# ScissorJack-ever/AlayaLite

Hardware: AMD Instinct MI355X
Metric: QPS @ recall@10>=0.95, GIST-960 L2, 1M base / 1k queries (higher is better)
Workload: dtype f32

## Files before the change

### alayalite_amd/csrc/capi.cpp

```cpp
#include "../../include/alaya_hip.h"

#include <hip/hip_runtime_api.h>

#include <algorithm>
#include <cfloat>
#include <cmath>
#include <cstring>
#include <memory>
#include <mutex>
#include <stdexcept>
#include <limits>
#include <string>
#include <thread>
#include <vector>

#include "build_kernels.h"
#include "extend_kernels.h"
#include "graph_update.h"
#include "hnsw_build.h"
#include "flat_bound.h"
#include "flat_filtered_kernels.h"
#include "flat_kernels.h"
#include <cstdlib>
#include "screen_bound.h"
// ... 73 lines not shown
  int device = 0;
  std::mutex mu;
  uint64_t n = 0;
  uint32_t dim = 0, stride = 0;
  int metric = ALAYA_METRIC_L2;
  bool generic = false;
  DevBuf base, valid;
  bool has_valid = false;
  bool has_graph = false;
  uint32_t R = 0, upper_R = 0, ep = 0, n_eps = 0;
  bool has_overlay = false, dedup = false;
  DevBuf l0, levels, upper_off, upper_edges, eps;
  uint64_t graph_n = 0;
  bool has_sq8 = false;
  int sq8_order = 2;
  uint32_t code_stride = 0;
  DevBuf codes, sq_min, sq_max, rr_q_buf, sq_ids, sq_d;
  DevBuf norms, cand_d, cand_i, flat_tau, flag_buf, iota, flat_q;
  DevBuf flat_bias;
  int flat_contraction = -1;
  bool norms_ready = false;
  DevBuf flat_tiles, tiles_cand, tiles_qexp;
  bool tiles_ready = false;
  int tiles_exp = 0;
  int tiles_metric = -1;
  float max_norm = 0.f;
  DevBuf work, overflow, dirty, stab, q_buf, id_buf, dist_buf, cnt_buf, dlist_buf, dout_buf;
  DevBuf allow_buf, group_buf;
  DevBuf through_buf;
  DevBuf ff_ids, ff_sums, ff_count, ff_part_d, ff_part_i, ff_qlist;
  uint64_t ff_last[4] = {0, 0, 0, 0};
  size_t overflow_clean = 0;
  size_t stab_clean = 0;
  uint32_t hash_log2_override = 0;
  int helpers_mode = -1;
  DevBuf help_stats;
  uint64_t help_stats_slots = 0;
  struct ScreenCopy {
    DevBuf rows, err;
    uint64_t cap = 0;
    bool ready = false;
    bool failed = false;
  };
  ScreenCopy screen_copy[2];
  uint32_t screen_format = 0;
  DevBuf screen_stats;
  uint64_t screen_stats_slots = 0;
  uint32_t last_grid = 0, last_waves = 0;
  uint32_t last_lds = 0, last_hash_log2 = 0, last_compact = 0, last_per_cu = 0, last_scout = 0;
  DevBuf scout_stats;
  uint64_t scout_stats_slots = 0;
  DevBuf scout_policy_stats;
  uint32_t last_scout_policy = 0;
  int visited_mode_override = 0;
  int num_cus = 0;
  uint64_t capacity = 0;
  std::unique_ptr<alaya_amd::HostGraph> upd_graph;
  std::unique_ptr<alaya_amd::RowMirror> upd_rows;
  std::unique_ptr<alaya_amd::UpdateContext> upd_ctx;
  hipStream_t stream = nullptr;
  hipEvent_t scratch_ev = nullptr;
  hipStream_t scratch_stream = nullptr;
  bool scratch_used = false;
  uint64_t device_bytes() const {
    return base.bytes + valid.bytes + l0.bytes + levels.bytes + upper_off.bytes +
           upper_edges.bytes + eps.bytes + overflow.bytes + dirty.bytes + stab.bytes + codes.bytes + sq_min.bytes +
           sq_max.bytes;
  }
};

namespace {

void set_device(const alaya_index *ix) { hip_check(hipSetDevice(ix->device), "hipSetDevice"); }

void scratch_acquire(alaya_index *ix, hipStream_t s) {
  if (ix->scratch_used && ix->scratch_stream != s)
    hip_check(hipStreamWaitEvent(s, ix->scratch_ev, 0), "hipStreamWaitEvent");
}
void scratch_release(alaya_index *ix, hipStream_t s) {
  hip_check(hipEventRecord(ix->scratch_ev, s), "hipEventRecord");
  ix->scratch_stream = s;
  ix->scratch_used = true;
}
void scratch_suspect(alaya_index *ix) {
  ix->overflow_clean = 0;
  ix->stab_clean = 0;
}
void scratch_drain(alaya_index *ix) {
  if (!ix->scratch_used) return;
  const hipError_t e = hipEventSynchronize(ix->scratch_ev);
  if (e != hipSuccess) scratch_suspect(ix);
  hip_check(e, "hipEventSynchronize");
}
template <typename F>
int guarded_scratch(alaya_index *ix, F &&f) {
  return guarded([&] {
    try {
      f();
    } catch (const DeviceError &) {
      if (ix) scratch_suspect(ix);
      throw;
    }
  });
}

SearchParams base_params(alaya_index *ix) {
// ... 185 lines not shown
  if (helpers_requested(ix, p, nq, static_cast<uint64_t>(stream_cus(ix, stream))) && ix->R <= 64 &&
      search_has_helpers(ix->dim, p.sq8_order, ix->generic))
    r.want |= kModeHelp;
  const bool plain = (r.want & (kModeHelp | kModeStamp)) == 0;
  if (plain && search_has_two_waves(ix->dim, p.sq8_order, ix->generic)) {
    const char *e = std::getenv("ALAYA_TWO_WAVES");
    const int force = e ? std::atoi(e) : -1;
    if (force == 1) {
      r.want |= kModeTwoWaves;
    } else if (force != 0) {
      int b1 = 0;
      const size_t probe = search_wave_lds_bytes(ix->stride, ef, 12, true);
      hip_check(search_occupancy(resolve_search_variant(r), p.ip, 1, probe, &b1), "occupancy");
      const uint64_t resident1 = static_cast<uint64_t>(std::max(1, b1)) * static_cast<uint64_t>(stream_cus(ix, stream));
      if (nq > resident1 && 2 * nq <= 3 * resident1) r.want |= kModeTwoWaves;
    }
  }
  if (ensure_screen(ix, p, p.sq8_order == 0 && plain, stream)) r.want |= kModeScreen;
  return r;
}

struct SearchPlan {
  const alaya_amd::SearchVariant *variant;
  int W;
  size_t lds;
  int grid;
  int per_cu;
};

uint32_t scout_default(uint32_t dim) { return (dim == 768 || dim == 960) ? alaya_amd::kScoutOn : 0u; }

uint32_t scout_requested(uint32_t dim) {
  const char *e = std::getenv("ALAYA_SEARCH_SCOUT");
  const int asked = e && e[0] ? std::atoi(e) : -1;
  uint32_t f = asked < 0 ? scout_default(dim) : (asked == 1 ? alaya_amd::kScoutOn : (asked == 2 ? alaya_amd::kScoutOn | alaya_amd::kScoutVerify : 0u));
  if (f != 0u) {
    const char *m = std::getenv("ALAYA_SEARCH_SCOUT_MISS");
    if (m && std::atoi(m) != 0) f |= alaya_amd::kScoutMiss;
  }
  return f;
}

uint32_t scout_policy_default(uint32_t dim) {
  return (dim == 768 || dim == 960) ? (alaya_amd::kScoutEarly | alaya_amd::kScoutRecheck) : 0u;
}

uint32_t scout_policy_requested(uint32_t dim) {
  const char *e = std::getenv("ALAYA_SEARCH_SCOUT_POLICY");
  if (!(e && e[0])) return scout_policy_default(dim);
  return static_cast<uint32_t>(std::strtoul(e, nullptr, 0)) &
         (alaya_amd::kScoutEarly | alaya_amd::kScoutRecheck);
}

SearchPlan plan_search(alaya_index *ix, SearchParams &p, alaya_amd::SearchRequest r, uint64_t nq, uint32_t ef,
                       hipStream_t stream) {
  using namespace alaya_amd;
  SearchPlan plan{};
  for (;;) {
    plan.variant = &resolve_search_variant(r);
    const int mode = plan.variant->mode;
    if ((r.want & kModeStamp) != 0 && (mode & kModeStamp) == 0)
      throw ArgError("no stamped search kernel for dim " + std::to_string(ix->dim) +
                     (p.sq8_order ? " SQ8 (order " + std::to_string(p.sq8_order) + ")" : std::string(" f32")) +
                     ": see the variant list in search_variants.h");
    p.help = (mode & kModeHelp) != 0;
    p.two_waves = (mode & kModeTwoWaves) != 0;
    p.screen = (mode & kModeScreen) != 0 ? ix->screen_format : 0u;
    plan.W = p.help ? 4 : search_waves(p);
    while (!p.help && plan.W > 1 && static_cast<uint64_t>(plan.W) > nq) plan.W /= 2;
    p.hash_log2 = size_visited(ix, p, *plan.variant, nq, ef, plan.W);
    const bool compact = p.vis_rbits != kVisWide;
    p.wave_lds = static_cast<uint32_t>(search_wave_lds_bytes(ix->stride, ef, p.hash_log2, compact, p.sq8_order));
    bool fits = true;
    if (p.help) {
      const size_t need = static_cast<size_t>(plan.W) * kHelpMemoSlots * ix->R * 8;
      const size_t q_bytes = search_query_lds_bytes(ix->stride, p.sq8_order);
      if (q_bytes >= need) {
        p.memo_off = 0;
      } else if (p.wave_lds >= q_bytes + 3 * 64 * 4 + need) {
        p.memo_off = static_cast<uint32_t>(q_bytes + 3 * 64 * 4);
      } else {
        fits = false;
      }
    }
    plan.lds = search_shared_lds_bytes(ix->stride, p.sq8_order != 0) + static_cast<size_t>(plan.W) * p.wave_lds +
               (p.help ? kHelpBoardBytes : 0);
    if (!p.help || (fits && plan.lds <= kLdsPerCu)) break;
    r.want &= ~kModeHelp;
  }
  if (plan.lds > kLdsPerCu) throw ArgError("ef / dim too large for the LDS budget");
  int per_cu = 0;
  hip_check(search_occupancy(*plan.variant, p.ip, plan.W, plan.lds, &per_cu), "occupancy");
  per_cu = static_cast<int>(std::max<uint64_t>(1, std::min<uint64_t>(per_cu, max_search_waves_per_cu() / plan.W)));
  const uint64_t cus = static_cast<uint64_t>(stream_cus(ix, stream));
  const uint64_t blocks_needed = p.help ? static_cast<uint64_t>(per_cu) * cus : (nq + plan.W - 1) / plan.W;
  plan.grid = static_cast<int>(std::max<uint64_t>(1, std::min<uint64_t>(blocks_needed, static_cast<uint64_t>(per_cu) * cus)));
  plan.per_cu = per_cu;
  p.scout = 0u;
  p.scout_policy = 0u;
  const uint32_t scout = scout_requested(ix->dim);
  if (scout != 0u && p.screen == 3u && !p.ip && !p.two_waves && !p.help && plan.W == 1 && ix->R <= kScoutR &&
      (plan.variant->mode & ~kModeScreen) == 0 && search_has_two_waves(ix->dim, p.sq8_order, ix->generic) &&
      !helpers_requested(ix, p, nq, cus)) {
    SearchRequest r2 = r;
    r2.want |= kModeTwoWaves;
    const SearchVariant &v2 = resolve_search_variant(r2);
    const size_t lds2 = plan.lds + kScoutBoardBytes;
    int per_cu2 = 0;
    if (v2.mode == (kModeScreen | kModeTwoWaves) && lds2 <= kLdsPerCu)
      hip_check(search_occupancy(v2, false, 2, lds2, &per_cu2), "occupancy");
    if (per_cu2 >= per_cu && nq <= static_cast<uint64_t>(per_cu) * cus) {
      plan.variant = &v2;
      plan.lds = lds2;
      p.scout = scout;
      p.scout_policy = scout_policy_requested(ix->dim);
      if (const char *e = std::getenv("ALAYA_SEARCH_SCOUT_GRID"))
        plan.grid = std::max(1, std::min(plan.grid, std::atoi(e)));
    }
  }
  return plan;
}

SearchParams graph_search_params(alaya_index *ix, const float *d_q, uint64_t nq, uint32_t k, uint32_t ef, uint32_t *d_ids,
                                 float *d_dists, uint32_t *d_cnt) {
  SearchParams p = base_params(ix);
  p.l0 = ix->l0.as<uint32_t>();
  p.R = ix->R;
  p.dedup_edges = ix->dedup;
  p.levels = ix->has_overlay ? ix->levels.as<uint32_t>() : nullptr;
  p.upper_off = ix->upper_off.as<uint64_t>();
  p.upper_edges = ix->upper_edges.as<uint32_t>();
  p.upper_R = ix->upper_R;
  p.ep = ix->ep;
  p.eps = ix->eps.as<uint32_t>();
  p.n_eps = ix->n_eps;
  p.queries = d_q;
  p.nq = nq;
  p.q_stride = ix->dim;
  p.k = k;
  p.ef = ef;
  p.out_ids = d_ids;
  p.out_dists = d_dists;
  p.out_counters = d_cnt;
  return p;
}

void set_search_space(alaya_index *ix, SearchParams &p, bool sq8, uint32_t ef) {
  if (sq8) {
    p.sq8_order = ix->sq8_order;
    p.codes = ix->codes.as<uint8_t>();
    p.code_stride = ix->code_stride;
    p.sq_min = ix->sq_min.as<float>();
    p.sq_max = ix->sq_max.as<float>();
  }
  p.stab_log2 = spill_table_log2(p.sq8_order, std::max<uint32_t>(1, ceil_log2(std::max<uint64_t>(ix->n, 2))), ef);
}

void record_launch(alaya_index *ix, SearchParams &p, int grid, int wg_waves, size_t lds, int per_cu, uint64_t searchers,
                   hipStream_t stream) {
  ix->last_grid = static_cast<uint32_t>(grid);
  ix->last_waves = static_cast<uint32_t>(wg_waves);
  ix->last_lds = static_cast<uint32_t>(lds);
  ix->last_hash_log2 = p.hash_log2;
  ix->last_compact = p.vis_rbits != alaya_amd::kVisWide ? 1u : 0u;
  ix->last_per_cu = static_cast<uint32_t>(per_cu);
  ix->last_scout = p.scout;
  ix->last_scout_policy = p.scout_policy;
  ix->scout_stats_slots = p.scout ? searchers : 0;
  ix->help_stats_slots = p.help ? searchers : 0;
  ix->screen_stats_slots = p.screen ? searchers : 0;
  ix->work.reserve(4);
  p.work_counter = ix->work.as<uint32_t>();
  hip_check(hipMemsetAsync(p.work_counter, 0, 4, stream), "hipMemsetAsync");
}

void do_search(alaya_index *ix, const float *d_q, uint64_t nq, uint32_t k, uint32_t ef,
               uint32_t *d_ids, float *d_dists, uint32_t *d_cnt, hipStream_t stream,
               uint64_t *d_stamps = nullptr, bool sq8 = false, uint32_t fill_id = 0) {
  if (!ix->base.ptr) throw ArgError("index has no base vectors");
  if (!ix->has_graph) throw ArgError("index has no graph");
  if (ef == 0) throw ArgError("ef must be >= 1");
  if (k == 0 || nq == 0) return;
  if (ix->graph_n > ix->n) throw ArgError("graph has more nodes than base vectors");
  SearchParams p = graph_search_params(ix, d_q, nq, k, ef, d_ids, d_dists, d_cnt);
  p.stamps = d_stamps;
  p.fill_id = fill_id;
  if (sq8 && !ix->has_sq8) throw ArgError("index has no SQ8 codes");
  set_search_space(ix, p, sq8, ef);
  if (const char *e = std::getenv("ALAYA_HELP_FLAGS")) p.help_flags = static_cast<uint32_t>(std::strtoul(e, nullptr, 10));
  const SearchPlan plan = plan_search(ix, p, search_request(ix, p, nq, ef, stream), nq, ef, stream);
  if (p.screen >= 2) {
    p.screen_u8 = ix->screen_copy[1].rows.as<uint8_t>();
  } else if (p.screen) {
    p.screen_rows = ix->screen_copy[0].rows.as<uint16_t>();
    p.screen_err = ix->screen_copy[0].err.as<float>();
  }
  scratch_acquire(ix, stream);
  const uint64_t searchers = static_cast<uint64_t>(plan.grid) * plan.W;
  prepare_spill(ix, p, searchers, stream);
  const int wg_waves = p.scout ? 2 * plan.W : plan.W;
  if (p.scout) {
    ix->scout_stats.reserve(searchers * 16);
    p.scout_stats = ix->scout_stats.as<uint32_t>();
    ix->scout_policy_stats.reserve(searchers * 12);
    p.scout_policy_stats = ix->scout_policy_stats.as<uint32_t>();
  }
  if (p.help) {
    ix->help_stats.reserve(searchers * 12);
    p.help_stats = ix->help_stats.as<uint32_t>();
  }
  if (p.screen) {
    ix->screen_stats.reserve(searchers * 8);
    p.screen_stats = ix->screen_stats.as<uint32_t>();
  }
  record_launch(ix, p, plan.grid, wg_waves, plan.lds, plan.per_cu, searchers, stream);
  hip_check(alaya_amd::launch_search(*plan.variant, p, plan.grid, wg_waves, plan.lds, stream), "search launch");
  scratch_release(ix, stream);
}

void do_filtered_search(alaya_index *ix, const float *d_q, uint64_t nq, uint32_t k, uint32_t ef, const uint32_t *d_allow,
// ... 1985 lines not shown
    if (waves_per_group) *waves_per_group = ix->last_waves;
  });
}

int alaya_index_last_plan(const alaya_index *ix, uint32_t *lds_bytes, uint32_t *hash_log2, uint32_t *compact,
                          uint32_t *groups_per_cu, uint32_t *scout) {
  return guarded([&] {
    if (!ix) throw ArgError("null index");
    if (lds_bytes) *lds_bytes = ix->last_lds;
    if (hash_log2) *hash_log2 = ix->last_hash_log2;
    if (compact) *compact = ix->last_compact;
    if (groups_per_cu) *groups_per_cu = ix->last_per_cu;
    if (scout) *scout = ix->last_scout;
  });
}

static std::vector<uint64_t> searcher_stats(alaya_index *ix, const DevBuf &buf, uint64_t searchers, uint32_t words) {
  std::vector<uint64_t> t(words, 0);
  if (searchers) {
    set_device(ix);
    scratch_drain(ix);
    std::vector<uint32_t> h(words * searchers);
    hip_check(hipMemcpy(h.data(), buf.ptr, h.size() * 4, hipMemcpyDeviceToHost), "D2H");
    for (uint64_t i = 0; i < h.size(); ++i) t[i % words] += h[i];
  }
  return t;
}

int alaya_index_scout_stats(alaya_index *ix, uint64_t *expansions, uint64_t *hits, uint64_t *records,
                            uint64_t *mismatches) {
  return guarded_scratch(ix, [&] {
    if (!ix) throw ArgError("null index");
    const std::vector<uint64_t> t = searcher_stats(ix, ix->scout_stats, ix->scout_stats_slots, 4);
    if (expansions) *expansions = t[0];
    if (hits) *hits = t[1];
    if (records) *records = t[2];
    if (mismatches) *mismatches = t[3];
  });
}

int alaya_index_scout_policy_stats(alaya_index *ix, uint32_t *policy, uint64_t *early_posts, uint64_t *confirmed,
                                   uint64_t *abandoned) {
  return guarded_scratch(ix, [&] {
    if (!ix) throw ArgError("null index");
    const bool sums = early_posts || confirmed || abandoned;
    const std::vector<uint64_t> t = searcher_stats(ix, ix->scout_policy_stats, sums ? ix->scout_stats_slots : 0, 3);
    if (policy) *policy = ix->last_scout_policy;
    if (early_posts) *early_posts = t[0];
    if (confirmed) *confirmed = t[1];
    if (abandoned) *abandoned = t[2];
  });
}

int alaya_index_set_helpers(alaya_index *ix, int mode) {
  return guarded([&] {
    if (!ix) throw ArgError("null index");
    if (mode < -1 || mode > 1) throw ArgError("helpers mode must be -1 (automatic), 0 (off) or 1 (on)");
    ix->helpers_mode = mode;
  });
}

int alaya_index_help_stats(alaya_index *ix, uint64_t *memo_dists, uint64_t *memo_expansions, uint64_t *helper_rows) {
  return guarded_scratch(ix, [&] {
    if (!ix) throw ArgError("null index");
    const std::vector<uint64_t> t = searcher_stats(ix, ix->help_stats, ix->help_stats_slots, 3);
    if (memo_dists) *memo_dists = t[0];
    if (memo_expansions) *memo_expansions = t[1];
    if (helper_rows) *helper_rows = t[2];
  });
}

int alaya_screen_lower_bound(const float *d_tilde, const float *e_row, uint64_t n, uint32_t dim, float *out) {
  return guarded([&] {
    if (n && (!d_tilde || !e_row || !out)) throw ArgError("invalid arguments");
    for (uint64_t i = 0; i < n; ++i) out[i] = alaya_amd::screen_lower_bound(d_tilde[i], e_row[i], dim);
  });
}

namespace {
void screen_u8_quantize_one(const float *x, uint32_t dim, uint8_t *codes, float *header, float *values) {
  using namespace alaya_amd;
  float lo = FLT_MAX, hi = -FLT_MAX;
  bool bad = false;
  for (uint32_t j = 0; j < dim; ++j) {
    bad = bad || !screen_finite(x[j]);
    lo = fminf(lo, x[j]);
    hi = fmaxf(hi, x[j]);
  }
  float scale = screen_u8_scale(lo, hi);
  if (bad || !screen_finite(scale)) {
    bad = true;
    lo = scale = 0.f;
  }
  float sum = 0.f;
  for (uint32_t j = 0; j < dim; ++j) {
    const uint32_t c = screen_u8_code(x[j], lo, scale);
    const float y = screen_u8_value(c, lo, scale);
    const float d = x[j] - y;
    if (!bad) sum = fmaf(d, d, sum);
    codes[j] = static_cast<uint8_t>(c);
    if (values) values[j] = y;
  }
  header[0] = screen_u8_err(sum, dim, bad);
  header[1] = lo;
  header[2] = scale;
  header[3] = 0.f;
// ... 115 lines not shown
```

### alayalite_amd/csrc/pybind_module.cpp

```cpp
#include <pybind11/numpy.h>
#include <pybind11/pybind11.h>
#include <pybind11/stl.h>

#include <algorithm>
#include <cmath>
#include <cstring>
#include <fstream>
#include <memory>
#include <queue>
#include <stdexcept>
#include <string>
#include <vector>

#include "../../include/alaya_hip.h"

extern "C" int alaya_index_flat_diag(alaya_index *, const float *, uint64_t, uint32_t, int, uint32_t *, float *,
                                     uint32_t *, uint32_t *, void *);
#include "host_distance.h"

namespace py = pybind11;

namespace alaya_py {

enum class IndexType { FLAT = 0, HNSW = 1, NSG = 2, FUSION = 3, QG = 4 };
// ... 105 lines not shown
                           eps.mutable_data()));
  return py::make_tuple(l0, has_overlay ? py::object(levels) : py::none(), has_overlay ? py::object(off) : py::none(), ue,
                        ep, upper_R, eps);
}

class LaunchControls {
 public:
  void set_hash_log2(uint32_t v) { check(alaya_index_set_hash_log2(ix_, v)); }
  void set_visited_mode(int m) { check(alaya_index_set_visited_mode(ix_, m)); }
  void set_helpers(int m) { check(alaya_index_set_helpers(ix_, m)); }
  py::tuple last_launch() {
    uint32_t g = 0, w = 0;
    check(alaya_index_last_launch(ix_, &g, &w));
    return py::make_tuple(g, w);
  }
  py::tuple help_stats() {
    uint64_t m = 0, x = 0, r = 0;
    check(alaya_index_help_stats(ix_, &m, &x, &r));
    return py::make_tuple(m, x, r);
  }
  py::tuple screen_stats() {
    uint64_t a = 0, b = 0;
    check(alaya_index_screen_stats(ix_, &a, &b));
    return py::make_tuple(a, b);
  }
  py::tuple scout_stats() {
    uint64_t e = 0, h = 0, r = 0, m = 0;
    check(alaya_index_scout_stats(ix_, &e, &h, &r, &m));
    return py::make_tuple(e, h, r, m);
  }
  py::tuple scout_policy_stats() {
    uint64_t a = 0, c = 0, d = 0;
    check(alaya_index_scout_policy_stats(ix_, nullptr, &a, &c, &d));
    return py::make_tuple(a, c, d);
  }
  uint32_t scout_policy() {
    uint32_t pol = 0;
    check(alaya_index_scout_policy_stats(ix_, &pol, nullptr, nullptr, nullptr));
    return pol;
  }
  py::dict last_plan() {
    uint32_t g = 0, w = 0, lds = 0, hl = 0, c = 0, pc = 0, sc = 0;
    check(alaya_index_last_launch(ix_, &g, &w));
    check(alaya_index_last_plan(ix_, &lds, &hl, &c, &pc, &sc));
    py::dict d;
    d["workgroups"] = g;
    d["waves_per_group"] = w;
    d["lds_bytes"] = lds;
    d["hash_log2"] = hl;
    d["compact"] = c != 0;
    d["groups_per_cu"] = pc;
    d["scout"] = sc;
    d["scout_policy"] = scout_policy();
    return d;
  }

 protected:
  alaya_index *ix_ = nullptr;
};

class PyIndexInterface : public LaunchControls {
 public:
  explicit PyIndexInterface(const IndexParams &params) : params_(params) {
    dtype_ = dtype_code(params_.data_type_);
    if (params_.id_type_.is(py::dtype::of<uint32_t>())) {
      id_bytes_ = 4;
    } else if (params_.id_type_.is(py::dtype::of<uint64_t>())) {
      id_bytes_ = 8;
    } else {
      throw std::runtime_error("Unsupported id type");
    }
    if (params_.quantization_type_ == QuantizationType::SQ4 ||
        params_.quantization_type_ == QuantizationType::RABITQ)
      throw std::runtime_error("quantization type not supported by the MI355X engine (SQ4/RaBitQ are out of scope)");
    if (params_.metric_ == MetricType::COS && dtype_ != kF32 && dtype_ != kF64) {
      throw std::runtime_error("COS metric only support float or double");
    }
    if (params_.quantization_type_ == QuantizationType::SQ8 && dtype_ != kF32)
      throw std::runtime_error("SQ8 quantization of non-float32 data is not supported by the MI355X engine");
    check(alaya_index_create(0, &ix_));
  }
  ~PyIndexInterface() {
    if (graph_) alaya_graph_free(graph_);
    if (ix_) alaya_index_destroy(ix_);
  }
  PyIndexInterface(const PyIndexInterface &) = delete;
  PyIndexInterface &operator=(const PyIndexInterface &) = delete;

  std::string to_string() const { return "PyIndexInterface"; }

  void fit(py::array vectors, uint32_t ef_construction, uint32_t num_threads, const std::string &builder) {
    if (builder != "host" && builder != "gpu") throw py::value_error("builder must be 'host' or 'gpu'");
    if (vectors.ndim() != 2) throw std::runtime_error("Array must be 2D");
    check_dtype(vectors);
    py::array arr = py::array::ensure(vectors, py::array::c_style);
    const uint64_t n = arr.shape(0);
    dim_ = static_cast<uint32_t>(arr.shape(1));
    if (n > params_.capacity_) throw std::runtime_error("number of vectors exceeds the index capacity");
    if (params_.metric_ == MetricType::COS) normalize_in_place(arr, n);
    raw_.assign(static_cast<const char *>(arr.data()),
                static_cast<const char *>(arr.data()) + n * dim_ * dtype_size(dtype_));
    n_ = n;
    delete_cnt_ = 0;
    valid_.clear();
    rows_f32_.resize(n * dim_);
    to_float(raw_.data(), dtype_, n * dim_, rows_f32_.data());
// ... 1147 lines not shown
```

### alayalite_amd/csrc/search_device.h

```cpp
#pragma once
#include <hip/hip_runtime.h>

#include <cfloat>
#include <cstdint>

#include "screen_bound.h"
#include "search_kernels.h"

namespace alaya_amd {
namespace {

constexpr uint32_t kEmpty = 0xffffffffu;
constexpr uint32_t kChecked = 0x80000000u;
constexpr uint32_t kIdMask = 0x7fffffffu;

__device__ __forceinline__ int lane_id() { return __lane_id(); }

__device__ __forceinline__ void wave_sync() {
  __builtin_amdgcn_fence(__ATOMIC_SEQ_CST, "wavefront");
  __builtin_amdgcn_wave_barrier();
}

__device__ __forceinline__ uint64_t ballot(bool p) { return __ballot(p); }

// ... 1160 lines not shown
  if (lane_in_row && row_v != kEmpty)
    lo = __hip_atomic_load(&vs.bits[row_v >> 5], __ATOMIC_RELAXED, __HIP_MEMORY_SCOPE_AGENT);
}

__device__ __forceinline__ void visit_end(Visited &vs) {
  if (!vs.spilled) return;
  const int lane = lane_id();
  __threadfence_block();
  if (vs.stab != nullptr) {
    uint64_t *t = reinterpret_cast<uint64_t *>(vs.stab);
    const uint32_t n8 = 2u * (vs.stab_bmask + 1u);
    for (uint32_t i = lane; i < n8; i += 64) __hip_atomic_store(t + i, 0ull, __ATOMIC_RELAXED, ALAYA_STAB_SCOPE);
  }
  if (vs.ndirty <= vs.dirty_cap) {
    for (uint32_t i = lane; i < vs.ndirty; i += 64)
      __hip_atomic_store(&vs.bits[vs.dirty[i]], 0u, __ATOMIC_RELAXED, __HIP_MEMORY_SCOPE_AGENT);
  } else {
    for (uint64_t w = lane; w < vs.n_words; w += 64)
      __hip_atomic_store(&vs.bits[w], 0u, __ATOMIC_RELAXED, __HIP_MEMORY_SCOPE_AGENT);
  }
  stab_order();
  vs.spilled = false;
}

struct PoolState {
  uint32_t size;
  uint32_t cur;
  uint32_t ef;
};

__device__ __forceinline__ uint32_t pool_upper_bound(const float *pd, uint32_t size, float d) {
  uint32_t lo = 0, hi = size;
  while (lo < hi) {
    const uint32_t mid = (lo + hi) >> 1;
    if (pd[mid] > d) hi = mid; else lo = mid + 1;
  }
  return lo;
}

__device__ __forceinline__ uint32_t batch_lower_bound(const float *sd, uint32_t n, float d) {
  uint32_t lo = 0, hi = n;
  while (lo < hi) {
    const uint32_t mid = (lo + hi) >> 1;
    if (sd[mid] < d) lo = mid + 1; else hi = mid;
  }
  return lo;
}

struct NoNext {
  __device__ void operator()(uint32_t) const {}
};

struct NoMark {
  __device__ void operator()() const {}
};

template <bool kRegMerge = false, typename OnNext = NoNext, typename Mark = NoMark>
__device__ void pool_merge(PoolState &ps, const Lds &L, bool has, uint32_t id, float d,
                           OnNext on_next = OnNext(), Mark mark = Mark()) {
  const int lane = lane_id();
  const bool full = ps.size == ps.ef;
  const float last = full ? L.pd[ps.size - 1] : 0.f;
  const bool acc = has && !(full && d >= last);
  const uint64_t amask = ballot(acc);
  const uint32_t n_acc = __popcll(amask);
  if (n_acc == 0) return;
  if (kRegMerge && ps.ef <= 128) {
    const uint32_t size = ps.size;
    const bool v0 = static_cast<uint32_t>(lane) < size;
    const bool v1 = static_cast<uint32_t>(lane) + 64 < size;
    const float p0 = v0 ? L.pd[lane] : 0.f;
    const float p1 = v1 ? L.pd[lane + 64] : 0.f;
    const uint32_t i0 = v0 ? L.pi[lane] : 0u;
    const uint32_t i1 = v1 ? L.pi[lane + 64] : 0u;
    if (!ballot((acc && d != d) || (v0 && p0 != p0) || (v1 && p1 != p1))) {
      uint32_t rank = 0, pos = 0, s0 = 0, s1 = 0;
      uint64_t rest = amask;
      while (rest) {
        const int j = __ffsll(static_cast<unsigned long long>(rest)) - 1;
        rest &= rest - 1;
        const float dj = read_lane(d, j);
        rank += (dj < d || (dj == d && j < lane)) ? 1u : 0u;
        const uint32_t ub = __popcll(ballot(v0 && p0 <= dj)) + __popcll(ballot(v1 && p1 <= dj));
        if (lane == j) pos = ub;
        s0 += dj < p0 ? 1u : 0u;
        s1 += dj < p1 ? 1u : 0u;
      }
      pos += rank;
      const int lane0 = __ffsll(static_cast<unsigned long long>(ballot(acc && rank == 0))) - 1;
      const uint32_t first_pos = read_lane(pos, lane0);
      if (first_pos <= ps.cur) on_next(read_lane(id, lane0));
      mark();
      wave_sync();
      if (v0 && s0 != 0 && lane + s0 < ps.ef) {
        L.pd[lane + s0] = p0;
        L.pi[lane + s0] = i0;
      }
      if (v1 && s1 != 0 && lane + 64 + s1 < ps.ef) {
        L.pd[lane + 64 + s1] = p1;
        L.pi[lane + 64 + s1] = i1;
      }
      if (acc && pos < ps.ef) {
        L.pd[pos] = d;
        L.pi[pos] = id;
      }
      wave_sync();
      ps.size = min(size + n_acc, ps.ef);
      if (first_pos < ps.cur) ps.cur = first_pos;
      return;
    }
  }
  uint32_t rank = 0;
  uint64_t rest = amask;
#if ALAYA_PAIR_LOOPS
  while (rest) {
    const int j = __ffsll(static_cast<unsigned long long>(rest)) - 1;
    rest &= rest - 1;
    const bool t2 = rest != 0ull;
    const int j2 = t2 ? __ffsll(static_cast<unsigned long long>(rest)) - 1 : j;
    rest &= t2 ? rest - 1 : rest;
    const float dj = read_lane(d, j);
    const float dj2 = read_lane(d, j2);
    rank += (dj < d || (dj == d && j < lane)) ? 1u : 0u;
    rank += (t2 && (dj2 < d || (dj2 == d && j2 < lane))) ? 1u : 0u;
  }
#else
  while (rest) {
    const int j = __ffsll(static_cast<unsigned long long>(rest)) - 1;
    rest &= rest - 1;
    const float dj = read_lane(d, j);
    rank += (dj < d || (dj == d && j < lane)) ? 1u : 0u;
  }
#endif
  if (acc) L.sd[rank] = d;
  uint32_t pos = 0;
  if (acc) pos = pool_upper_bound(L.pd, ps.size, d) + rank;
  const int lane0 = __ffsll(static_cast<unsigned long long>(ballot(acc && rank == 0))) - 1;
  const uint32_t first_pos = read_lane(pos, lane0);
  if (first_pos <= ps.cur) on_next(read_lane(id, lane0));
  mark();
  wave_sync();
  for (int hi = static_cast<int>(ps.size); hi > static_cast<int>(first_pos); hi -= 64) {
    const int j = hi - 64 + lane;
    const bool mv = j >= static_cast<int>(first_pos);
    float pdj = 0.f;
    uint32_t pij = 0;
    uint32_t dest = 0;
    if (mv) {
      pdj = L.pd[j];
      pij = L.pi[j];
      dest = static_cast<uint32_t>(j) + batch_lower_bound(L.sd, n_acc, pdj);
    }
    wave_sync();
    if (mv && dest < ps.ef) {
      L.pd[dest] = pdj;
      L.pi[dest] = pij;
    }
    wave_sync();
  }
  if (acc && pos < ps.ef) {
    L.pd[pos] = d;
    L.pi[pos] = id;
  }
  wave_sync();
  ps.size = min(ps.size + n_acc, ps.ef);
  if (first_pos < ps.cur) ps.cur = first_pos;
}

template <bool kNext = false>
__device__ __forceinline__ uint32_t pool_pop(PoolState &ps, const Lds &L, uint32_t *c1 = nullptr,
                                             uint32_t *c2 = nullptr) {
  const int lane = lane_id();
  const uint32_t raw = L.pi[ps.cur];
  wave_sync();
  if (lane == 0) L.pi[ps.cur] = raw | kChecked;
  uint32_t next = ps.size;
  if constexpr (kNext) *c1 = *c2 = kEmpty;
  for (uint32_t b = ps.cur + 1; b < ps.size; b += 64) {
    const uint32_t j = b + lane;
    const uint32_t pij = j < ps.size ? L.pi[j] : kChecked;
    const bool un = !(pij & kChecked);
    const uint64_t mk = ballot(un);
    if (mk) {
      const int f = __ffsll(static_cast<unsigned long long>(mk)) - 1;
      next = b + f;
      if constexpr (kNext) {
        *c1 = read_lane(pij & kIdMask, f);
        const uint64_t mk2 = mk & (mk - 1ull);
        if (mk2) *c2 = read_lane(pij & kIdMask, __ffsll(static_cast<unsigned long long>(mk2)) - 1);
      }
      break;
    }
  }
  wave_sync();
  ps.cur = next;
  return raw & kIdMask;
}

}
}
```

### alayalite_amd/csrc/search_kernels.h

```cpp
#pragma once
#include <hip/hip_runtime_api.h>

#include <cstddef>
#include <cstdint>

#include "search_variants.h"

namespace alaya_amd {

struct SearchParams {
  const float *base;
  uint64_t n;
  uint32_t dim;
  uint32_t stride;
  const uint32_t *valid;
  bool ip;
  bool generic;
  const uint32_t *l0;
  uint32_t R;
  bool dedup_edges;
  const uint32_t *levels;
  const uint64_t *upper_off;
  const uint32_t *upper_edges;
  uint32_t upper_R;
  uint32_t ep;
  const uint32_t *eps;
  uint32_t n_eps;
  const float *queries;
  uint64_t nq;
  uint32_t q_stride;
  uint32_t k;
  uint32_t ef;
  uint32_t *out_ids;
  float *out_dists;
  uint32_t *out_counters;
  uint32_t fill_id;
  uint32_t *work_counter;
  uint32_t *overflow_bits;
  uint32_t *dirty_words;
  uint32_t dirty_cap;
  uint32_t wave_lds;
  uint32_t hash_log2;
  uint32_t vis_rbits;
  uint32_t vis_lbits;
  uint32_t vis_max_disp;
  uint32_t vis_limit;
  uint16_t *spill_table;
  uint32_t stab_log2;
  uint32_t stab_rbits;
  uint32_t spill_flags;
  uint64_t *stamps;
  int sq8_order;
  const uint8_t *codes;
  uint32_t code_stride;
  const float *sq_min;
  const float *sq_max;
  uint32_t help;
  uint32_t help_flags;
  uint32_t memo_off;
  uint32_t two_waves;
  uint32_t *help_stats;
  uint32_t screen;
  const uint16_t *screen_rows;
  const float *screen_err;
  const uint8_t *screen_u8;
  uint32_t *screen_stats;
  uint32_t scout;
  uint32_t *scout_stats;
  uint32_t scout_policy;
  uint32_t *scout_policy_stats;
};
constexpr uint32_t kScoutOn = 1, kScoutVerify = 2, kScoutMiss = 4;
constexpr uint32_t kScoutEarly = 1, kScoutRecheck = 2;
constexpr uint32_t kScoutSlots = 3;
constexpr uint32_t kScoutR = 32;
constexpr size_t kScoutBoardBytes = kScoutSlots * (kScoutR * 4 + 8 + 4) + 20;

struct FilterParams {
  const uint32_t *allow;
  const uint32_t *mask_of_query;
  uint32_t mask_words;
  uint32_t k;
  uint32_t result_off;
};

struct HopParams {
  uint32_t *n_through;
};

struct RerankParams {
  const uint32_t *search_ids;
  uint32_t k;
  uint32_t n_src;
  uint32_t n_take;
  uint32_t zeros;
  uint32_t fill_id;
  uint32_t *out_ids;
  float *out_dists;
};

constexpr uint32_t kVisWide = 0xffffffffu;
constexpr size_t kHelpBoardBytes = 256;
#ifndef ALAYA_HELP_DEPTH
#define ALAYA_HELP_DEPTH 1
#endif
constexpr size_t kHelpMemoSlots = ALAYA_HELP_DEPTH + 1;
constexpr uint32_t kStabBucket = 8;
inline size_t visited_table_bytes(uint32_t hash_log2, bool compact) {
  return (static_cast<size_t>(compact ? 2 : 4)) << hash_log2;
}
size_t search_wave_lds_bytes(uint32_t stride, uint32_t ef, uint32_t hash_log2, bool compact = false,
                             int sq8_order = 0);
size_t search_query_lds_bytes(uint32_t stride, int sq8_order);
__host__ __device__ inline size_t search_shared_lds_bytes(uint32_t stride, bool sq8) {
  return sq8 ? 2 * static_cast<size_t>(stride) * 4 : 0;
}
hipError_t launch_rerank(const SearchParams &p, const RerankParams &r, hipStream_t stream);
hipError_t search_occupancy(const SearchVariant &v, bool ip, int waves, size_t lds, int *blocks_per_cu);
hipError_t launch_screen_rows(const float *base, uint64_t first, uint64_t count, uint32_t stride,
                              uint16_t *out_rows, float *out_err, hipStream_t stream);
hipError_t launch_screen_rows_u8(const float *base, uint64_t first, uint64_t count, uint32_t stride,
                                 uint8_t *out_recs, hipStream_t stream);
hipError_t launch_search(const SearchVariant &v, const SearchParams &p, int grid, int waves, size_t lds,
                         hipStream_t stream);
size_t filter_result_lds_bytes(uint32_t k);
hipError_t filtered_search_occupancy(uint32_t dim, bool generic, bool ip, int waves, size_t lds, int *blocks_per_cu);
// ... 17 lines not shown
```

### alayalite_amd/csrc/search_kernels.hip

```cpp
#include <hip/hip_runtime.h>

#include <cfloat>
#include <cstdint>

#include "screen_bound.h"
#include "search_kernels.h"
#include "search_device.h"

#ifndef ALAYA_MIN_WAVES_SQ8
#define ALAYA_MIN_WAVES_SQ8 -1
#endif
#ifndef ALAYA_MIN_WAVES_NARROW
#define ALAYA_MIN_WAVES_NARROW 0
#endif
#ifndef ALAYA_MIN_WAVES_WIDE
#define ALAYA_MIN_WAVES_WIDE 0
#endif
template <int kSpace>
constexpr bool space_sq8() { return kSpace == 1 || kSpace == 2; }
template <int kSpace>
constexpr bool space_tab() { return kSpace == 2; }

template <int kChunks, int kSpace, int kMode = 0>
constexpr int search_min_waves() {
// ... 920 lines not shown
            const float4 head = *reinterpret_cast<const float4 *>(rp);
            const uint2 sums = *reinterpret_cast<const uint2 *>(rp + screen_u8_sums_offset(p.stride));
            screen_dots_int<kChunks>(p, sq.codes, L.cid, nf, reinterpret_cast<uint32_t *>(L.cd), second_level_prefetch);
            lb3 = screen_int_bound(p.stride, sq.err, sq.lo, sq.scale, sq.a1, sq.a2, head.x, head.y, head.z, sums.x, sums.y,
                                   __float_as_uint(L.cd[lane]));
          } else if (p.screen == 2) {
            if (in) e_row = *reinterpret_cast<const float *>(p.screen_u8 + static_cast<uint64_t>(c) * screen_u8_record_bytes(p.stride));
            screen_distances_u8<kChunks, kScreenRowsU8>(p, L.q, L.cid, nf, L.cd, second_level_prefetch);
          } else {
            if (in) e_row = p.screen_err[c];
            screen_distances<kChunks, kScreenRows>(p, L.q, L.cid, nf, L.cd, second_level_prefetch);
          }
          bool keep = false;
          if (in) {
            const float lb = p.screen == 3 ? lb3 : screen_lower_bound(L.cd[lane], e_row, p.dim);
            keep = !(lb > 0.f && lb >= tau);
          }
          const uint64_t km = ballot(keep);
          nd = __popcll(km);
          n_screened += static_cast<uint32_t>(nf);
          n_screened_out += static_cast<uint32_t>(nf - nd);
          if constexpr (kScout) {
            if (early && nd > 0 && ps.cur < ps.size) scout_early_request(sboard, L, ps, keep, lb3, c, pred);
          }
          if (keep) L.cid[__popcll(km & ((1ull << lane) - 1ull))] = c;
          wave_sync();
          if (nd == 0) {
            stamp(3);
            n_dist += nf;
            continue;
          }
        }
      }
      if constexpr (kScreen) {
        constexpr int kFull = RowPass<kChunks, kRows>::kR;
        if (nd <= 8) {
          space_distances<kIP, kChunks, kSpace, false, 1>(p, L, L.cid, nd, L.cd);
        } else if (kFull > 2 && nd <= 16) {
          space_distances<kIP, kChunks, kSpace, false, 2>(p, L, L.cid, nd, L.cd);
        } else {
          space_distances<kIP, kChunks, kSpace, false, kRows>(p, L, L.cid, nd, L.cd);
        }
      } else if (!kHelp || compute) {
        space_distances<kIP, kChunks, kSpace, kHelp, kRows>(p, L, dist_ids, nf, L.cd, second_level_prefetch);
      } else {
        second_level_prefetch();
      }
      stamp(3);
      n_dist += nf;
      const bool has = lane < nd;
      const uint32_t cid = has ? L.cid[lane] : 0u;
      const float cd = has ? L.cd[lane] : 0.f;
      wave_sync();
      pool_merge<kRegMerge>(ps, L, has, cid, cd, [&](uint32_t nx) {
        if (nx != pred) {
          const uint32_t old_pred = pred;
          (void)old_pred;
          pred = nx;
          if (lane < static_cast<int>(p.R)) pred_v = p.l0[static_cast<uint64_t>(nx) * p.R + lane];
          if constexpr (kHelp) {
            if (mine.memo_wave >= 0) mine_request(board, wave, mine, kEmpty, nx, old_pred);
          }
          if constexpr (kScout) {
            if (scouting && ps.size == ps.ef) scout_retarget(sboard, early, nx, old_pred);
          }
        }
      }
#ifdef ALAYA_FINE_STAMPS
      , [&]() { stamp(7); }
#endif
      );
      stamp(4);
    }

    query_end(p, L, ps, qi, n_dist, n_expand, n_dist_up, n_hops_up);
    visit_end(vs);
    if constexpr (kStamp) {
      st[6] = __builtin_readcyclecounter() - t_begin;
      if (lane < 8) p.stamps[static_cast<uint64_t>(qi) * 8 + lane] = st[lane & 7];
    }
    wave_sync();
  }
  if constexpr (kHelp) {
    help_siblings<kIP, kChunks, kSpace>(p, smem, L, board, wave, W);
    help_stats_out(p, board, wave, slot, lane);
  }
  if constexpr (kScout) {
    if (scouting) scout_leave(p, sboard, slot);
  }
  if constexpr (kScreen) screen_stats_out(p, slot, n_screened, n_screened_out, lane);
}

__global__ void __launch_bounds__(256) screen_rows_kernel(const float *base, uint64_t first, uint64_t count,
                                                          uint32_t stride, uint16_t *out_rows, float *out_err) {
  const int lane = lane_id();
  const uint64_t waves = static_cast<uint64_t>(gridDim.x) * (blockDim.x >> 6);
  for (uint64_t r = static_cast<uint64_t>(blockIdx.x) * (blockDim.x >> 6) + (threadIdx.x >> 6); r < count; r += waves) {
    const float *row = base + (first + r) * stride;
    uint16_t *dst = out_rows + (first + r) * stride;
    float sum = 0.f;
    bool bad = false;
    for (uint32_t e = 2 * lane; e < stride; e += 128) {
      const float2 x = *reinterpret_cast<const float2 *>(row + e);
      const _Float16 h0 = static_cast<_Float16>(x.x), h1 = static_cast<_Float16>(x.y);
      const float y0 = static_cast<float>(h0), y1 = static_cast<float>(h1);
      bad = bad || !(fabsf(y0) <= 65504.f) || !(fabsf(y1) <= 65504.f) || !(fabsf(x.x) <= FLT_MAX) ||
            !(fabsf(x.y) <= FLT_MAX);
      const float d0 = x.x - y0, d1 = x.y - y1;
      sum = fmaf(d0, d0, sum);
      sum = fmaf(d1, d1, sum);
      const half2_t h = {h0, h1};
      *reinterpret_cast<uint32_t *>(dst + e) = __builtin_bit_cast(uint32_t, h);
    }
    sum += lane_xor<1>(sum);
    sum += lane_xor<2>(sum);
    sum += lane_xor<4>(sum);
    sum += lane_xor<8>(sum);
    sum += lane_xor<16>(sum);
    sum = read_lane(sum, 0) + read_lane(sum, 32);
    const bool any_bad = ballot(bad) != 0ull;
    if (lane == 0) {
      float err = sqrtf(sum * (1.0f + screen_gamma(stride))) * (1.0f + 1.9073486328125e-6f) + 8.8817841970012523e-16f;
      if (any_bad || !(err <= kScreenHuge)) err = __builtin_inff();
      out_err[first + r] = err;
// ... 770 lines not shown
```

### include/alaya_hip.h

```cpp
#ifndef ALAYA_HIP_H_
#define ALAYA_HIP_H_

#include <stddef.h>
#include <stdint.h>

#ifdef __cplusplus
extern "C" {
#endif

#define ALAYA_OK 0
#define ALAYA_ERR_ARG 1
#define ALAYA_ERR_RUNTIME 2
#define ALAYA_ERR_DEVICE 3

#define ALAYA_METRIC_L2 0
#define ALAYA_METRIC_IP 1
#define ALAYA_METRIC_COS 2
#define ALAYA_DIST_GENERIC 0x100

typedef struct alaya_index alaya_index;
typedef struct alaya_graph alaya_graph;

const char *alaya_last_error(void);
const char *alaya_build_info(void);
// ... 83 lines not shown
int alaya_sq8_encode(const float *data, uint64_t n, uint32_t dim, const float *min_v,
                     const float *max_v, uint8_t *codes, uint32_t num_threads);
int alaya_index_set_sq8(alaya_index *ix, const uint8_t *codes, uint64_t n, uint32_t dim,
                        const float *min_v, const float *max_v, int order);
int alaya_index_batch_search_sq8(alaya_index *ix, const float *queries, const float *rerank_queries,
                                 uint64_t nq, uint32_t k, uint32_t ef, int rerank, uint32_t *ids,
                                 float *dists, uint32_t *counters);
int alaya_index_batch_search_sq8_device(alaya_index *ix, const float *d_queries, const float *d_rerank_queries,
                                        uint64_t nq, uint32_t k, uint32_t ef, int rerank, uint32_t *d_ids,
                                        float *d_dists, uint32_t *d_counters, void *stream);
int alaya_index_shard_search_sq8_device(alaya_index *ix, const float *d_queries, const float *d_rerank_queries,
                                        uint64_t nq, uint32_t k, uint32_t ef, int holds_row0, uint32_t *d_ids,
                                        float *d_dists, uint32_t *d_counters, void *stream);
int alaya_index_flat_search(alaya_index *ix, const float *queries, uint64_t nq, uint32_t k,
                            uint32_t *ids, float *dists, uint32_t *n_recomputed);
int alaya_index_flat_search_device(alaya_index *ix, const float *d_queries, uint64_t nq, uint32_t k,
                                   uint32_t *d_ids, float *d_dists, uint32_t *d_flags, void *stream);
int alaya_index_flat_last_contraction(const alaya_index *ix, int *contraction);
int alaya_index_flat_search_filtered(alaya_index *ix, const float *queries, uint64_t nq, uint32_t k,
                                     const uint32_t *allow_words, uint32_t n_masks, const uint32_t *mask_of_query,
                                     uint32_t *ids, float *dists);
int alaya_index_flat_search_filtered_device(alaya_index *ix, const float *d_queries, uint64_t nq, uint32_t k,
                                            const uint32_t *d_allow_words, uint32_t n_masks,
                                            const uint32_t *d_mask_of_query, uint32_t *d_ids, float *d_dists,
                                            void *stream);
int alaya_index_flat_filtered_last(const alaya_index *ix, uint64_t *out);
int alaya_flat_filtered_plan(uint64_t n_allowed, uint64_t nq, uint32_t k, uint32_t stride, uint32_t cus,
                             uint64_t *out);
int alaya_index_set_hash_log2(alaya_index *ix, uint32_t log2_slots);
int alaya_index_set_visited_mode(alaya_index *ix, int mode);
int alaya_index_set_helpers(alaya_index *ix, int mode);
int alaya_index_help_stats(alaya_index *ix, uint64_t *memo_dists, uint64_t *memo_expansions,
                           uint64_t *helper_rows);
int alaya_index_screen_stats(alaya_index *ix, uint64_t *screened, uint64_t *screened_out);
int alaya_screen_lower_bound(const float *d_tilde, const float *e_row, uint64_t n, uint32_t dim, float *out);
int alaya_screen_u8_quantize(const float *rows, uint64_t n, uint32_t dim, uint8_t *codes, float *header,
                             float *values);
int alaya_screen_int_bound(const float *queries, const float *rows, uint64_t n, uint32_t dim, float *d_in,
                           float *e_sum, float *bound, uint32_t *sums);
int alaya_flat_ip_slack(int contraction, uint32_t k_acc, const float *q_norm2, const int *q_exp, uint64_t n,
                        float b_max, int base_exp, float *out);
int alaya_flat_ip_proven(const float *kth_d, const float *cutoff, const float *slack, uint64_t n, uint8_t *out);
int alaya_search_variant(uint32_t dim, int ip, int sq8_order, int generic, uint32_t wanted_mode, int *space,
                         uint32_t *chunks, uint32_t *mode, uint32_t *has_mode);
int alaya_search_variant_at(uint32_t index, int *space, uint32_t *chunks, uint32_t *mode, int *l2_only,
                            uint32_t *count);
int alaya_index_last_launch(const alaya_index *ix, uint32_t *workgroups, uint32_t *waves_per_group);
int alaya_index_last_plan(const alaya_index *ix, uint32_t *lds_bytes, uint32_t *hash_log2, uint32_t *compact,
                          uint32_t *groups_per_cu, uint32_t *scout);
int alaya_index_scout_stats(alaya_index *ix, uint64_t *expansions, uint64_t *hits, uint64_t *records,
                            uint64_t *mismatches);
int alaya_index_scout_policy_stats(alaya_index *ix, uint32_t *policy, uint64_t *early_posts, uint64_t *confirmed,
                                   uint64_t *abandoned);
int alaya_index_info(const alaya_index *ix, uint64_t *n, uint32_t *dim, uint32_t *stride,
                     int *metric, uint64_t *device_bytes);

#ifdef __cplusplus
}
#endif
#endif
```

Before: 350,600.

## Add register-resident wide pool merge for full pools with ef 129-448

Adds a wide merge path to pool_merge. Once the candidate pool is full, each lane holds seven pool distances in registers. Insert positions and per-slot shift counts come from ballots and packed byte counters, replacing the binary search plus the chunked LDS shifting loop. It is on by default for dim 960 screen or stamp variants when ef is in range, and can be toggled with an environment variable. This adds register pressure and extra loop work per accepted candidate, and falls back to the old path on NaNs.

```diff
diff --git a/alayalite_amd/csrc/capi.cpp b/alayalite_amd/csrc/capi.cpp
--- a/alayalite_amd/csrc/capi.cpp
+++ b/alayalite_amd/csrc/capi.cpp
@@ -149,6 +149,7 @@
   uint64_t scout_stats_slots = 0;
   DevBuf scout_policy_stats;
   uint32_t last_scout_policy = 0;
+  uint32_t last_wide_merge = 0;
   int visited_mode_override = 0;
   int num_cus = 0;
   uint64_t capacity = 0;
@@ -440,6 +441,15 @@
          (alaya_amd::kScoutEarly | alaya_amd::kScoutRecheck);
 }
 
+uint32_t wide_merge_default(uint32_t dim) { return dim == 960 ? 1u : 0u; }
+
+uint32_t wide_merge_requested(uint32_t dim, uint32_t ef) {
+  if (ef < alaya_amd::kWideMergeMinEf || ef > alaya_amd::kWideMergeMaxEf) return 0u;
+  const char *e = std::getenv("ALAYA_SEARCH_WIDE_MERGE");
+  if (!(e && e[0])) return wide_merge_default(dim);
+  return std::atoi(e) != 0 ? 1u : 0u;
+}
+
 SearchPlan plan_search(alaya_index *ix, SearchParams &p, alaya_amd::SearchRequest r, uint64_t nq, uint32_t ef,
                        hipStream_t stream) {
   using namespace alaya_amd;
@@ -506,6 +516,7 @@
         plan.grid = std::max(1, std::min(plan.grid, std::atoi(e)));
     }
   }
+  p.wide_merge = (plan.variant->mode & (kModeScreen | kModeStamp)) != 0 ? wide_merge_requested(ix->dim, ef) : 0u;
   return plan;
 }
 
@@ -554,6 +565,7 @@
   ix->last_per_cu = static_cast<uint32_t>(per_cu);
   ix->last_scout = p.scout;
   ix->last_scout_policy = p.scout_policy;
+  ix->last_wide_merge = p.screen ? p.wide_merge : 0u;
   ix->scout_stats_slots = p.scout ? searchers : 0;
   ix->help_stats_slots = p.help ? searchers : 0;
   ix->screen_stats_slots = p.screen ? searchers : 0;
@@ -2645,6 +2657,13 @@
   });
 }
 
+int alaya_index_last_wide_merge(const alaya_index *ix, uint32_t *wide_merge) {
+  return guarded([&] {
+    if (!ix) throw ArgError("null index");
+    if (wide_merge) *wide_merge = ix->last_wide_merge;
+  });
+}
+
 int alaya_index_set_helpers(alaya_index *ix, int mode) {
   return guarded([&] {
     if (!ix) throw ArgError("null index");
diff --git a/alayalite_amd/csrc/pybind_module.cpp b/alayalite_amd/csrc/pybind_module.cpp
--- a/alayalite_amd/csrc/pybind_module.cpp
+++ b/alayalite_amd/csrc/pybind_module.cpp
@@ -181,6 +181,9 @@
     d["groups_per_cu"] = pc;
     d["scout"] = sc;
     d["scout_policy"] = scout_policy();
+    uint32_t wm = 0;
+    check(alaya_index_last_wide_merge(ix_, &wm));
+    d["wide_merge"] = wm;
     return d;
   }
 
diff --git a/alayalite_amd/csrc/search_device.h b/alayalite_amd/csrc/search_device.h
--- a/alayalite_amd/csrc/search_device.h
+++ b/alayalite_amd/csrc/search_device.h
@@ -1236,12 +1236,15 @@
 };
 
 struct NoMark {
-  __device__ void operator()() const {}
+  __device__ void operator()(uint32_t, uint32_t) const {}
 };
 
-template <bool kRegMerge = false, typename OnNext = NoNext, typename Mark = NoMark>
+constexpr int kWideRegs = 7;
+static_assert(kWideMergeMaxEf == 64 * kWideRegs, "the wide merge holds the whole pool");
+
+template <bool kRegMerge = false, bool kWide = false, typename OnNext = NoNext, typename Mark = NoMark>
 __device__ void pool_merge(PoolState &ps, const Lds &L, bool has, uint32_t id, float d,
-                           OnNext on_next = OnNext(), Mark mark = Mark()) {
+                           OnNext on_next = OnNext(), Mark mark = Mark(), bool wide = false) {
   const int lane = lane_id();
   const bool full = ps.size == ps.ef;
   const float last = full ? L.pd[ps.size - 1] : 0.f;
@@ -1274,7 +1277,7 @@
       const int lane0 = __ffsll(static_cast<unsigned long long>(ballot(acc && rank == 0))) - 1;
       const uint32_t first_pos = read_lane(pos, lane0);
       if (first_pos <= ps.cur) on_next(read_lane(id, lane0));
-      mark();
+      mark(first_pos, n_acc);
       wave_sync();
       if (v0 && s0 != 0 && lane + s0 < ps.ef) {
         L.pd[lane + s0] = p0;
@@ -1294,61 +1297,197 @@
       return;
     }
   }
-  uint32_t rank = 0;
-  uint64_t rest = amask;
+  if constexpr (!kWide) {
+    uint32_t rank = 0;
+    uint64_t rest = amask;
 #if ALAYA_PAIR_LOOPS
-  while (rest) {
-    const int j = __ffsll(static_cast<unsigned long long>(rest)) - 1;
-    rest &= rest - 1;
-    const bool t2 = rest != 0ull;
-    const int j2 = t2 ? __ffsll(static_cast<unsigned long long>(rest)) - 1 : j;
-    rest &= t2 ? rest - 1 : rest;
-    const float dj = read_lane(d, j);
-    const float dj2 = read_lane(d, j2);
-    rank += (dj < d || (dj == d && j < lane)) ? 1u : 0u;
-    rank += (t2 && (dj2 < d || (dj2 == d && j2 < lane))) ? 1u : 0u;
-  }
+    while (rest) {
+      const int j = __ffsll(static_cast<unsigned long long>(rest)) - 1;
+      rest &= rest - 1;
+      const bool t2 = rest != 0ull;
+      const int j2 = t2 ? __ffsll(static_cast<unsigned long long>(rest)) - 1 : j;
+      rest &= t2 ? rest - 1 : rest;
+      const float dj = read_lane(d, j);
+      const float dj2 = read_lane(d, j2);
+      rank += (dj < d || (dj == d && j < lane)) ? 1u : 0u;
+      rank += (t2 && (dj2 < d || (dj2 == d && j2 < lane))) ? 1u : 0u;
+    }
 #else
-  while (rest) {
-    const int j = __ffsll(static_cast<unsigned long long>(rest)) - 1;
-    rest &= rest - 1;
-    const float dj = read_lane(d, j);
-    rank += (dj < d || (dj == d && j < lane)) ? 1u : 0u;
-  }
+    while (rest) {
+      const int j = __ffsll(static_cast<unsigned long long>(rest)) - 1;
+      rest &= rest - 1;
+      const float dj = read_lane(d, j);
+      rank += (dj < d || (dj == d && j < lane)) ? 1u : 0u;
+    }
 #endif
-  if (acc) L.sd[rank] = d;
-  uint32_t pos = 0;
-  if (acc) pos = pool_upper_bound(L.pd, ps.size, d) + rank;
-  const int lane0 = __ffsll(static_cast<unsigned long long>(ballot(acc && rank == 0))) - 1;
-  const uint32_t first_pos = read_lane(pos, lane0);
-  if (first_pos <= ps.cur) on_next(read_lane(id, lane0));
-  mark();
-  wave_sync();
-  for (int hi = static_cast<int>(ps.size); hi > static_cast<int>(first_pos); hi -= 64) {
-    const int j = hi - 64 + lane;
-    const bool mv = j >= static_cast<int>(first_pos);
-    float pdj = 0.f;
-    uint32_t pij = 0;
-    uint32_t dest = 0;
-    if (mv) {
-      pdj = L.pd[j];
-      pij = L.pi[j];
-      dest = static_cast<uint32_t>(j) + batch_lower_bound(L.sd, n_acc, pdj);
-    }
+    if (acc) L.sd[rank] = d;
+    uint32_t pos = 0;
+    if (acc) pos = pool_upper_bound(L.pd, ps.size, d) + rank;
+    const int lane0 = __ffsll(static_cast<unsigned long long>(ballot(acc && rank == 0))) - 1;
+    const uint32_t first_pos = read_lane(pos, lane0);
+    if (first_pos <= ps.cur) on_next(read_lane(id, lane0));
+    mark(first_pos, n_acc);
     wave_sync();
-    if (mv && dest < ps.ef) {
-      L.pd[dest] = pdj;
-      L.pi[dest] = pij;
+    for (int hi = static_cast<int>(ps.size); hi > static_cast<int>(first_pos); hi -= 64) {
+      const int j = hi - 64 + lane;
+      const bool mv = j >= static_cast<int>(first_pos);
+      float pdj = 0.f;
+      uint32_t pij = 0;
+      uint32_t dest = 0;
+      if (mv) {
+        pdj = L.pd[j];
+        pij = L.pi[j];
+        dest = static_cast<uint32_t>(j) + batch_lower_bound(L.sd, n_acc, pdj);
+      }
+      wave_sync();
+      if (mv && dest < ps.ef) {
+        L.pd[dest] = pdj;
+        L.pi[dest] = pij;
+      }
+      wave_sync();
+    }
+    if (acc && pos < ps.ef) {
+      L.pd[pos] = d;
+      L.pi[pos] = id;
     }
     wave_sync();
-  }
-  if (acc && pos < ps.ef) {
-    L.pd[pos] = d;
-    L.pi[pos] = id;
-  }
-  wave_sync();
-  ps.size = min(ps.size + n_acc, ps.ef);
-  if (first_pos < ps.cur) ps.cur = first_pos;
+    ps.size = min(ps.size + n_acc, ps.ef);
+    if (first_pos < ps.cur) ps.cur = first_pos;
+  } else {
+    bool went_wide = false;
+    const uint32_t ef = ps.ef;
+    uint32_t base = 0;
+    float pw[kWideRegs] = {};
+    uint32_t sh_lo = 0, sh_hi = 0;
+    uint32_t pos = 0;
+    uint32_t first_pos = 0;
+    int lane0 = 0;
+    if constexpr (kWide) {
+      if (wide && full && ef >= kWideMergeMinEf && ef <= kWideMergeMaxEf) {
+        base = static_cast<uint32_t>(kWideRegs) * static_cast<uint32_t>(lane);
+        asm volatile("" : "+v"(base));
+        bool nan = acc && d != d;
+#pragma unroll
+        for (int r = 0; r < kWideRegs; ++r) {
+          pw[r] = L.pd[min(base + r, ef - 1u)];
+          nan = nan || pw[r] != pw[r];
+        }
+        if (!ballot(nan)) {
+          went_wide = true;
+          float first_d = 0.f;
+          lane0 = -1;
+          uint64_t rest = amask;
+          while (rest) {
+            const int j = __ffsll(static_cast<unsigned long long>(rest)) - 1;
+            rest &= rest - 1;
+            const float dj = read_lane(d, j);
+            pos += (dj < d || (dj == d && j < lane)) ? 1u : 0u;
+            uint32_t m = 0;
+#pragma unroll
+            for (int r = 0; r < kWideRegs; ++r) m |= dj < pw[r] ? 1u << r : 0u;
+            sh_lo += __umul24(m & 15u, 0x204081u) & 0x01010101u;
+            sh_hi += __umul24(m >> 4, 0x204081u) & 0x00010101u;
+            const uint32_t above = __popc(m);
+            const uint32_t lanes_le = __popcll(ballot(pw[0] <= dj));
+            const int b = lanes_le ? static_cast<int>(lanes_le) - 1 : 0;
+            const uint32_t ub = lanes_le ? static_cast<uint32_t>(kWideRegs) * lanes_le - read_lane(above, b) : 0u;
+            if (lane == j) pos += ub;
+            if (lane0 < 0 || dj < first_d) {
+              first_d = dj;
+              lane0 = j;
+              first_pos = ub;
+            }
+          }
+        }
+      }
+    }
+    if (!kWide || !went_wide) {
+      uint32_t rank = 0;
+      uint64_t rest = amask;
+#if ALAYA_PAIR_LOOPS
+      while (rest) {
+        const int j = __ffsll(static_cast<unsigned long long>(rest)) - 1;
+        rest &= rest - 1;
+        const bool t2 = rest != 0ull;
+        const int j2 = t2 ? __ffsll(static_cast<unsigned long long>(rest)) - 1 : j;
+        rest &= t2 ? rest - 1 : rest;
+        const float dj = read_lane(d, j);
+        const float dj2 = read_lane(d, j2);
+        rank += (dj < d || (dj == d && j < lane)) ? 1u : 0u;
+        rank += (t2 && (dj2 < d || (dj2 == d && j2 < lane))) ? 1u : 0u;
+      }
+#else
+      while (rest) {
+        const int j = __ffsll(static_cast<unsigned long long>(rest)) - 1;
+        rest &= rest - 1;
+        const float dj = read_lane(d, j);
+        rank += (dj < d || (dj == d && j < lane)) ? 1u : 0u;
+      }
+#endif
+      if (acc) L.sd[rank] = d;
+      if (acc) pos = pool_upper_bound(L.pd, ps.size, d) + rank;
+      lane0 = __ffsll(static_cast<unsigned long long>(ballot(acc && rank == 0))) - 1;
+      first_pos = read_lane(pos, lane0);
+    }
+    if (first_pos <= ps.cur) on_next(read_lane(id, lane0));
+    mark(first_pos, n_acc);
+    wave_sync();
+    if constexpr (kWide) {
+      if (went_wide) {
+        asm volatile("" : "+v"(base));
+        auto dest_of = [&](int r) {
+          const uint32_t s = __builtin_amdgcn_ubfe(r < 4 ? sh_lo : sh_hi, 8u * (r & 3), 8u);
+          const uint32_t dest = base + r + s;
+          return s != 0 && dest < ef ? dest : kEmpty;
+        };
+#pragma unroll
+        for (int r = 0; r < kWideRegs; ++r) {
+          const uint32_t dest = dest_of(r);
+          if (dest != kEmpty) L.pd[dest] = pw[r];
+        }
+        if (acc && pos < ef) L.pd[pos] = d;
+        asm volatile("" : "+v"(base));
+        uint32_t iw[kWideRegs];
+#pragma unroll
+        for (int r = 0; r < kWideRegs; ++r) iw[r] = L.pi[min(base + r, ef - 1u)];
+        wave_sync();
+#pragma unroll
+        for (int r = 0; r < kWideRegs; ++r) {
+          const uint32_t dest = dest_of(r);
+          if (dest != kEmpty) L.pi[dest] = iw[r];
+        }
+        if (acc && pos < ef) L.pi[pos] = id;
+        wave_sync();
+        if (first_pos < ps.cur) ps.cur = first_pos;
+        return;
+      }
+    }
+    for (int hi = static_cast<int>(ps.size); hi > static_cast<int>(first_pos); hi -= 64) {
+      const int j = hi - 64 + lane;
+      const bool mv = j >= static_cast<int>(first_pos);
+      float pdj = 0.f;
+      uint32_t pij = 0;
+      uint32_t dest = 0;
+      if (mv) {
+        pdj = L.pd[j];
+        pij = L.pi[j];
+        dest = static_cast<uint32_t>(j) + batch_lower_bound(L.sd, n_acc, pdj);
+      }
+      wave_sync();
+      if (mv && dest < ps.ef) {
+        L.pd[dest] = pdj;
+        L.pi[dest] = pij;
+      }
+      wave_sync();
+    }
+    if (acc && pos < ps.ef) {
+      L.pd[pos] = d;
+      L.pi[pos] = id;
+    }
+    wave_sync();
+    ps.size = min(ps.size + n_acc, ps.ef);
+    if (first_pos < ps.cur) ps.cur = first_pos;
+  }
 }
 
 template <bool kNext = false>
diff --git a/alayalite_amd/csrc/search_kernels.h b/alayalite_amd/csrc/search_kernels.h
--- a/alayalite_amd/csrc/search_kernels.h
+++ b/alayalite_amd/csrc/search_kernels.h
@@ -68,10 +68,13 @@
   uint32_t scout;
   uint32_t *scout_stats;
   uint32_t scout_policy;
+  uint32_t wide_merge;
   uint32_t *scout_policy_stats;
 };
+static_assert(sizeof(SearchParams) == 392, "a field that grows SearchParams moves every kernel's hidden arguments");
 constexpr uint32_t kScoutOn = 1, kScoutVerify = 2, kScoutMiss = 4;
 constexpr uint32_t kScoutEarly = 1, kScoutRecheck = 2;
+constexpr uint32_t kWideMergeMinEf = 129, kWideMergeMaxEf = 448;
 constexpr uint32_t kScoutSlots = 3;
 constexpr uint32_t kScoutR = 32;
 constexpr size_t kScoutBoardBytes = kScoutSlots * (kScoutR * 4 + 8 + 4) + 20;
diff --git a/alayalite_amd/csrc/search_kernels.hip b/alayalite_amd/csrc/search_kernels.hip
--- a/alayalite_amd/csrc/search_kernels.hip
+++ b/alayalite_amd/csrc/search_kernels.hip
@@ -996,7 +996,7 @@
       const uint32_t cid = has ? L.cid[lane] : 0u;
       const float cd = has ? L.cd[lane] : 0.f;
       wave_sync();
-      pool_merge<kRegMerge>(ps, L, has, cid, cd, [&](uint32_t nx) {
+      auto retarget = [&](uint32_t nx) {
         if (nx != pred) {
           const uint32_t old_pred = pred;
           (void)old_pred;
@@ -1009,11 +1009,36 @@
             if (scouting && ps.size == ps.ef) scout_retarget(sboard, early, nx, old_pred);
           }
         }
-      }
+      };
 #ifdef ALAYA_FINE_STAMPS
-      , [&]() { stamp(7); }
+      auto merge_mark = [&](uint32_t first_pos, uint32_t n_acc) {
+        stamp(7);
+        if constexpr (kStamp) {
+          auto bump = [&](uint32_t c, uint64_t by) {
+            constexpr int slot_of[7] = {0, 1, 2, 3, 4, 5, 7};
+#pragma unroll
+            for (uint32_t s = 0; s < 7; ++s)
+              st[slot_of[s]] += (c == 2 * s ? by << 32 : 0ull) + (c == 2 * s + 1 ? by << 48 : 0ull);
+          };
+          const uint32_t trips = (ps.size - first_pos + 63u) / 64u;
+          bump(n_acc <= 2 ? n_acc - 1 : (n_acc <= 4 ? 2u : (n_acc <= 8 ? 3u : 4u)), 1);
+          bump(5u + (trips < 7u ? trips : 7u), 1);
+          bump(13u, n_acc);
+        }
+      };
+#else
+      const NoMark merge_mark;
 #endif
-      );
+#ifdef ALAYA_FINE_STAMPS
+      constexpr bool kWideMerge = kScreen || kStamp;
+#else
+      constexpr bool kWideMerge = kScreen;
+#endif
+      if constexpr (kWideMerge) {
+        pool_merge<kRegMerge, true>(ps, L, has, cid, cd, retarget, merge_mark, p.wide_merge != 0u);
+      } else {
+        pool_merge<kRegMerge>(ps, L, has, cid, cd, retarget, merge_mark);
+      }
       stamp(4);
     }
 
diff --git a/include/alaya_hip.h b/include/alaya_hip.h
--- a/include/alaya_hip.h
+++ b/include/alaya_hip.h
@@ -159,6 +159,7 @@
                             uint64_t *mismatches);
 int alaya_index_scout_policy_stats(alaya_index *ix, uint32_t *policy, uint64_t *early_posts, uint64_t *confirmed,
                                    uint64_t *abandoned);
+int alaya_index_last_wide_merge(const alaya_index *ix, uint32_t *wide_merge);
 int alaya_index_info(const alaya_index *ix, uint64_t *n, uint32_t *dim, uint32_t *stride,
                      int *metric, uint64_t *device_bytes);
 
```

Result: faster. 355,700, median of 6 (+1.5%).
